# chiefchewie/thu-acg-f2024-path-tracer

Hardware: AMD Instinct MI355X
Metric: Msamples/s (WxHxspp/s), scene 6 FHD@4000spp (higher is better)
Workload: dtype f64; 1 GPU; scene 6 (reference main.rs scene script: bunny+spot+cow OBJ meshes, envmap) 1920x1080 @ 4000 spp, max_depth 50, seed 1; parallelism=single GPU (1-rank communicator, no collective), slots_per_pixel=0, device= (gfx950:sramecc+:xnack-)

## Files before the change

include/pt_amd.h:

```cpp
#ifndef PT_AMD_H
#define PT_AMD_H
#include <stdint.h>
#ifdef __cplusplus
extern "C" {
#endif

typedef struct pt_ctx pt_ctx;
typedef struct pt_scene pt_scene;

typedef struct pt_camera {
    double aspect_ratio;
    uint32_t image_width, samples_per_pixel, max_depth, env_is_map;
    double vfov;
    double look_from[3], look_at[3], vup[3];
    double blur_strength, focal_length, defocus_angle;
    double env_color[3];
    int32_t env_tex;
    int32_t _pad;
} pt_camera;

typedef struct pt_render_opts {
    uint32_t slots_per_pixel;
    uint32_t accum_on_device;
    uint32_t profile;
    uint32_t overwrite;
    void* stream;
} pt_render_opts;

typedef struct pt_render_stats {
    uint64_t samples, segments, iterations;
    uint32_t n_slots, slots_per_pixel;
    double ms_total;
    double ms_extend, ms_shade, ms_other;
    uint64_t launches_extend, launches_shade;
    uint32_t extend_variant, shade_variant;
    uint32_t blocks_extend, blocks_shade;
    uint32_t compactions;
    uint32_t n_alloc_end;
    uint64_t short_direct_tiles, short_self_prims;
    uint64_t short_walks, short_walk_passes;
    uint64_t pilot_tiles, short_fallback, short_list_bytes, short_pixels;
    double ms_pilot;
    uint64_t short_tiles, short_samples, hard_samples;
    double ms_short;
    uint64_t sky_tiles, sky_samples;
    double ms_sky;
} pt_render_stats;

const char* pt_last_error(void);
int pt_set_error_message(const char* msg);
int pt_ctx_create(int device, pt_ctx** out);
void pt_ctx_destroy(pt_ctx*);
int pt_device_name(pt_ctx*, char* buf, uint32_t n);
// ... 236 lines not shown
```

thu-acg-f2024-path-tracer_amd/__init__.py:

```python
from __future__ import annotations

import ctypes as C
import math
import os
from typing import Optional, Sequence

import numpy as np

_HERE = os.path.dirname(os.path.abspath(__file__))
REPO_ROOT = os.path.dirname(_HERE)
LIB_PATH = os.environ.get("PT_AMD_LIB") or os.path.join(_HERE, "libpt_amd.so")
ASSET_DIR = os.path.join(REPO_ROOT, "assets")


class PtError(RuntimeError):
    pass


class Camera(C.Structure):

    _fields_ = [
        ("aspect_ratio", C.c_double),
        ("image_width", C.c_uint32),
        ("samples_per_pixel", C.c_uint32),
# ... 29 lines not shown
        ("iterations", C.c_uint64),
        ("n_slots", C.c_uint32),
        ("slots_per_pixel", C.c_uint32),
        ("ms_total", C.c_double),
        ("ms_extend", C.c_double),
        ("ms_shade", C.c_double),
        ("ms_other", C.c_double),
        ("launches_extend", C.c_uint64),
        ("launches_shade", C.c_uint64),
        ("extend_variant", C.c_uint32),
        ("shade_variant", C.c_uint32),
        ("blocks_extend", C.c_uint32),
        ("blocks_shade", C.c_uint32),
        ("compactions", C.c_uint32),
        ("n_alloc_end", C.c_uint32),
        ("short_direct_tiles", C.c_uint64),
        ("short_self_prims", C.c_uint64),
        ("short_walks", C.c_uint64),
        ("short_walk_passes", C.c_uint64),
        ("pilot_tiles", C.c_uint64),
        ("short_fallback", C.c_uint64),
        ("short_list_bytes", C.c_uint64),
        ("short_pixels", C.c_uint64),
        ("ms_pilot", C.c_double),
        ("short_tiles", C.c_uint64),
        ("short_samples", C.c_uint64),
        ("hard_samples", C.c_uint64),
        ("ms_short", C.c_double),
        ("sky_tiles", C.c_uint64),
        ("sky_samples", C.c_uint64),
# ... 1181 lines not shown
```

thu-acg-f2024-path-tracer_amd/csrc/pt_k2.hip:

```cpp
#include "pt_k2_extend.h"

namespace pt {

typedef void (*extend_fn)(SceneD, PoolD, CountersD*);
static extend_fn pick_extend2(int code) {
    switch (code) {
    case 163: return k_extend2<16, 3>;
    case 164: return k_extend2<16, 4>;
    case 204: return k_extend2<20, 4>;
    case 283: return k_extend2<28, 3>;
    case 323: return k_extend2<32, 3>;
    case 1164: return k_extend2<16, 4, 64>;
    case 2164: return k_extend2<16, 4, 128>;
    case 8164: return k_extend2<16, 4, 512>;
    default: return k_extend2<24, 3>;
    }
}
static extend_fn pick_extend2_mot(int code) {
    const int stack = (code % 1000) / 10;
    if (stack <= 16) return k_extend2<16, 4, 128, true>;
    if (stack <= 20) return k_extend2<20, 4, BLOCK, true>;
    if (stack <= 24) return k_extend2<24, 3, BLOCK, true>;
    if (stack <= 28) return k_extend2<28, 3, BLOCK, true>;
    return k_extend2<32, 3, BLOCK, true>;
}
static int extend2_threads(int code) { return code >= 1000 ? (code / 1000) * 64 : BLOCK; }
static int extend2_threads_mot(int code) { return (code % 1000) / 10 <= 16 ? 128 : BLOCK; }
static extend_fn pick_extend_batch(uint32_t flat, uint32_t pairs, bool motion = false) {
    if (motion) return !flat ? k_extend<false, false, true> : pairs ? k_extend<true, true, true> : k_extend<true, false, true>;
    return !flat ? k_extend<false, false> : pairs ? k_extend<true, true> : k_extend<true, false>;
}
void launch_extend(const SceneD& sc, const PoolD& pool, CountersD* cnt, int max_blocks, int code, hipStream_t st, bool motion) {
    if (code <= -100) {
        const int kb = motion ? extend2_threads_mot(-code) : extend2_threads(-code);
        const uint32_t blocks = clamp_blocks(pool.n_alloc / (uint32_t)(EXT_WINDOW / BLOCK * kb), max_blocks);
        hipLaunchKernelGGL(motion ? pick_extend2_mot(-code) : pick_extend2(-code), dim3(blocks), dim3((uint32_t)kb), 0, st, sc, pool, cnt);
    }
    else hipLaunchKernelGGL(pick_extend_batch(sc.tlas_flat, sc.flat_pairs, motion), grid_for(pool.n_alloc, max_blocks), dim3(BLOCK), 0, st, sc, pool, cnt);
}
int extend_occupancy_blocks(int code, bool motion) {
    if (code <= -100) return motion ? occupancy_blocks((const void*)pick_extend2_mot(-code), extend2_threads_mot(-code))
                                    : occupancy_blocks((const void*)pick_extend2(-code), extend2_threads(-code));
    return occupancy_blocks((const void*)pick_extend_batch(code <= -2, code == -3, motion), BLOCK);
}

}
```

thu-acg-f2024-path-tracer_amd/csrc/pt_k2_extend.h:

```cpp
#pragma once
#include "pt_k_trace.h"

namespace pt {

#ifndef PT_EXTEND_BATCH_BLOCKS
#define PT_EXTEND_BATCH_BLOCKS 4
#endif

#ifndef PT_PAIR_DENSE_MIN
#define PT_PAIR_DENSE_MIN 16
#endif
#ifndef PT_PAIR_PASS_ATTR
#define PT_PAIR_PASS_ATTR PT_DEV
#endif
#ifndef PT_FLAT_DIRECT
#define PT_FLAT_DIRECT 1
#endif
#ifndef PT_CUBOID_CULL
#define PT_CUBOID_CULL 1
#endif
#ifndef PT_PAIR_SINGLE
#define PT_PAIR_SINGLE 1
#endif
constexpr int PAIR_CAP = 128;
// ... 203 lines not shown
constexpr int EXT_WINDOW = 2048;
#ifndef PT_REFILL_MIN
#define PT_REFILL_MIN 16
#endif
constexpr uint32_t REFILL_MIN = PT_REFILL_MIN;
#ifndef PT_EXT_CAND
#define PT_EXT_CAND 768
#endif
#ifndef PT_EXT_CAND_SMALL
#define PT_EXT_CAND_SMALL 1024
#endif
constexpr int EXT_CAND = PT_EXT_CAND, EXT_CAND_SMALL = PT_EXT_CAND_SMALL;
static_assert(EXT_WINDOW % BLOCK == 0 && EXT_WINDOW <= 65536, "k_extend2: s_cand_sl holds 16-bit slot offsets inside the window");
static_assert(EXT_WINDOW == SORT_WINDOW_SLOTS, "the pool is allocated in whole windows of this size (pt_render.cpp rounds n_alloc to 2048)");

template <int EXT_STACK, int MINB, int KB = BLOCK, bool MOT = false>
__global__ __launch_bounds__(KB, MINB) void k_extend2(SceneD sc, PoolD pool, CountersD* cnt) {
    constexpr int WIN = EXT_WINDOW / BLOCK * KB, CAND = (KB <= 128 ? EXT_CAND_SMALL : EXT_CAND) / BLOCK * KB;
    __shared__ uint32_t stack[EXT_STACK * KB];
    __shared__ uint32_t s_best_id[WIN];
    __shared__ double s_cand_t[CAND];
    __shared__ uint32_t s_cand_items[CAND];
    __shared__ uint16_t s_cand_sl[CAND];
    __shared__ uint32_t s_nrays, s_next, s_win;
    uint32_t* stk = &stack[threadIdx.x];
    const int lane = (int)(threadIdx.x & 63u);
    const double t_min = 1e-3;
    const float t_min_f = __double2float_rd(t_min);
    unsigned long long nseg = 0;
    const uint32_t n_windows = pool.n_alloc / WIN;
    constexpr uint32_t PARTS = PT_TAIL_SPLIT ? PT_TAIL_PARTS : 1, CH = (uint32_t)(WIN / KB) / PARTS;
    static_assert(PARTS * CH == (uint32_t)(WIN / KB), "");
    const uint32_t n_tail = PT_TAIL_SPLIT ? (n_windows < gridDim.x * PT_TAIL_SPAN ? n_windows : gridDim.x * PT_TAIL_SPAN) : 0u;
    const uint32_t n_full = n_windows - n_tail, n_queue = n_full + PARTS * n_tail;
    if (blockIdx.x == 0 && threadIdx.x == 0) cnt->win_shade = 0;
    if (ldu(&cnt->alive) == 0ull) return;
#ifdef PT_STAMPS
    if (threadIdx.x < 8) g_prof[CLASS_DEAD][threadIdx.x] = 0ull;
#endif
    if (threadIdx.x == 0) { s_win = (uint32_t)atomicAdd(&cnt->win_extend, 1ull); s_nrays = 0; s_next = 0; }
    __syncthreads();
    for (;;) {
        const uint32_t q = s_win;
        if (q >= n_queue) break;
        const uint32_t win = q < n_full ? q : n_full + (q - n_full) / PARTS;
        const int j_lo = q < n_full ? 0 : (int)(((q - n_full) % PARTS) * CH), j_hi = q < n_full ? WIN / KB : j_lo + (int)CH;
        const uint32_t wbase = (PT_K2_REVERSE ? n_windows - 1u - win : win) * WIN;
        PT_STAMP(e0);
#if PT_K2_PREFETCH
        uint32_t state_next = pool.bounce[wbase + (uint32_t)j_lo * KB + threadIdx.x];
        RayD r_next{};
        if (state_next < SLOT_IDLE) r_next = load_ray(pool, wbase + (uint32_t)j_lo * KB + threadIdx.x);
#endif
        for (int j = j_lo; j < j_hi; ++j) {
            const uint32_t sl = (uint32_t)j * KB + threadIdx.x;
#if PT_K2_PREFETCH
            const uint32_t state = state_next;
            const bool alive = state < SLOT_IDLE;
            const RayD r = r_next;
            if (j + 1 < j_hi) {
                state_next = pool.bounce[wbase + sl + KB];
                if (state_next < SLOT_IDLE) r_next = load_ray(pool, wbase + sl + KB);
            }
#else
            const uint32_t state = pool.bounce[wbase + sl];
            const bool alive = state < SLOT_IDLE;
            RayD r{};
            if (alive) r = load_ray(pool, wbase + sl);
#endif
            uint32_t n_my = 0, items = 0xFFFFFFFFu;
            RayF f{};
            Closest best{D_INF, HIT_NONE};
            float t_max_f = t_max_f32(best.t);
            if (alive) {
                ++nseg;
                f = make_rayf(r.o, r.d, sc.tlas_extent);
            }
            auto visit_entry = [&](auto uniform, uint32_t ei, const Entry& e, int sp) {
                constexpr bool U = decltype(uniform)::value;
                if (e.kind == ENTRY_MESH) {
                    if (n_my < 4u && ei < 0xFFu) {
                        items = (items & ~(0xFFu << (8u * n_my))) | (ei << (8u * n_my));
                        ++n_my;
                    } else {
                        blas_pass<KB, MOT>(sc, r, e, t_min, t_min_f, stk + (size_t)sp * KB, EXT_STACK - sp, best);
                        t_max_f = t_max_f32(best.t);
                    }
                } else {
                    const RayD lr = ray_to_local_chain<U, MOT>(sc, e.inst, r);
                    const uint32_t n = e.kind == ENTRY_CUBOID ? 6u : 1u;
                    for (uint32_t i = 0; i < n; ++i) test_world_prim<U>(sc, lr, t_min, e.first_prim + i, best);
                    t_max_f = t_max_f32(best.t);
                }
            };
            if (sc.tlas_flat) {
                best = flat_top_level<false, true, MOT>(sc, alive, r, f, t_min, t_min_f, lane, PairLds{}, [&](uint32_t ei, const Entry& e, Closest& b) {
                    best = b;
                    visit_entry(std::true_type{}, ei, e, 0);
                    b = best;
                });
            } else if (alive) {
                int sp = 0;
                uint32_t cur = sc.tlas_root;
                for (;;) {
                    if ((cur & REF_TYPE_MASK) == REF_NODE) {
                        uint32_t c0, c1;
                        const int n = visit_node(&sc.nodes[cur], f, t_min_f, t_max_f, c0, c1);
                        if (n == 2 && sp < EXT_STACK) stk[(sp++) * KB] = c1;
                        if (n > 0) {
                            cur = c0;
                            continue;
                        }
                    } else if ((cur & REF_TYPE_MASK) == REF_ENTRY) {
                        const uint32_t ei = cur & 0x3FFFFFFFu;
                        visit_entry(std::false_type{}, ei, sc.entries[ei], sp);
                    }
                    if (sp == 0) break;
                    cur = stk[(--sp) * KB];
                }
            }
            const unsigned long long m = __ballot(n_my > 0);
            if (m) {
                const int leader = __ffsll((long long)m) - 1;
                uint32_t base = 0;
                if (lane == leader) base = atomicAdd(&s_nrays, (uint32_t)__popcll(m));
                base = (uint32_t)__shfl((int)base, leader);
                if (n_my > 0) {
                    const uint32_t pos = base + (uint32_t)__popcll(m & ((1ull << lane) - 1ull));
                    if (pos < (uint32_t)CAND) {
                        s_cand_t[pos] = best.t;
                        s_cand_items[pos] = items;
                        s_cand_sl[pos] = (uint16_t)sl;
                    } else {
                        for (uint32_t k = 0; k < n_my; ++k) blas_pass<KB, MOT>(sc, r, sc.entries[(items >> (8u * k)) & 0xFFu], t_min, t_min_f, stk, EXT_STACK, best);
                    }
                }
            }
            s_best_id[sl] = alive ? best.id : dead_or_idle(state);
        }
        PT_STAMP(e1);
        __syncthreads();
        PT_STAMP(e2);
        const uint32_t n_rays = s_nrays < (uint32_t)CAND ? s_nrays : (uint32_t)CAND;
        {
            bool busy = false, exhausted = false;
            uint32_t sl = 0, items = 0, item_k = 0, cur = REF_EMPTY, first_prim = 0;
            int sp = 0;
            RayD wr{}, r{};
            RayF f{};
            Closest best{D_INF, HIT_NONE};
            float t_max_f = 0.0f;
            auto start_item = [&]() -> bool {
                const uint32_t ei = item_k < 4u ? (items >> (8u * item_k)) & 0xFFu : 0xFFu;
                if (ei == 0xFFu) return false;
                const Entry e = sc.entries[ei];
                r = ray_to_local_chain<false, MOT>(sc, e.inst, wr);
                first_prim = e.first_prim;
                f = make_rayf(r.o, r.d, e.extent);
                t_max_f = t_max_f32(best.t);
// ... 37 lines not shown
                    if ((cur & REF_TYPE_MASK) == REF_TRIS) {
                        const uint32_t first = cur & 0x07FFFFFFu, count = ((cur >> 27) & 7u) + 1u;
                        test_leaf(sc, first, count, r, t_min, first_prim, best);
                        t_max_f = t_max_f32(best.t);
                        cur = sp > 0 ? stk[(--sp) * KB] : REF_EMPTY;
                    }
                    if (cur == REF_EMPTY) {
                        ++item_k;
                        if (!start_item()) {
                            s_best_id[sl] = best.id;
                            busy = false;
                        }
                    }
                }
            }
        }
        PT_STAMP(e3);
        __syncthreads();
        PT_STAMP(e4);
#ifdef PT_STAMPS
        if (lane == 0) {
            atomicAdd(&g_prof[CLASS_DEAD][0], 1ull);
            atomicAdd(&g_prof[CLASS_DEAD][1], t_e1 - t_e0);
            atomicAdd(&g_prof[CLASS_DEAD][2], t_e2 - t_e1);
            atomicAdd(&g_prof[CLASS_DEAD][3], t_e3 - t_e2);
            atomicAdd(&g_prof[CLASS_DEAD][4], t_e4 - t_e3);
            atomicAdd(&g_prof[CLASS_DEAD][5], (unsigned long long)n_rays);
        }
#endif
        {
            uint32_t word[WIN / KB];
#pragma unroll
            for (int j = 0; j < WIN / KB; ++j) word[j] = (j >= j_lo && j < j_hi) ? hit_word(sc, s_best_id[(uint32_t)j * KB + threadIdx.x]) : 0u;
#pragma unroll
            for (int j = 0; j < WIN / KB; ++j) if (j >= j_lo && j < j_hi) stnt(&pool.hit_prim[wbase + (uint32_t)j * KB + threadIdx.x], word[j]);
        }
        if (threadIdx.x == 0) { s_win = (uint32_t)atomicAdd(&cnt->win_extend, 1ull); s_nrays = 0; s_next = 0; }
        __syncthreads();
    }
    nseg = wave_sum(nseg);
    if (nseg && (threadIdx.x & 63u) == 0u) atomicAdd(&cnt->segments, nseg);
#ifdef PT_STAMPS
    __syncthreads();
    if (threadIdx.x < 8 && g_prof[CLASS_DEAD][threadIdx.x]) atomicAdd(&cnt->prof[CLASS_DEAD][threadIdx.x], g_prof[CLASS_DEAD][threadIdx.x]);
#endif
}

}
```

thu-acg-f2024-path-tracer_amd/csrc/pt_kernels.h:

```cpp
#pragma once
#include <hip/hip_runtime_api.h>

#include "pt_types.h"

namespace pt {
struct ShadeForm { int variant = 0; bool lights = false, list = false, qmc = false; ShadeMode mode = MODE_PLAIN; bool motion = false, punctual = false; };
ShadeForm shade_form(ShadeForm asked);
bool shade_form_sorts(const ShadeForm& form);
bool shade_form_maps_tiles(const ShadeForm& form);
bool launch_init(const CamD& cam, const PoolD& pool, uint64_t seed, int max_blocks, hipStream_t st, const ShadeForm& form);
void launch_extend(const SceneD& sc, const PoolD& pool, CountersD* cnt, int max_blocks, int code, hipStream_t st, bool motion = false);
bool launch_shade(const SceneD& sc, const CamD& cam, const PoolD& pool, CountersD* cnt, uint64_t seed, int max_blocks, const ShadeForm& form, hipStream_t st,
                  uint32_t wide_window_min = 16, const EnvTabD* env = nullptr);
int extend_occupancy_blocks(int code, bool motion = false);
int shade_occupancy_blocks(const ShadeForm& form);
void launch_medium_probe(int which, double density, double g, const double* in, uint32_t n, double* out, hipStream_t st);
void launch_grid_probe(int which, const GridD* grid, const float* vals, const double* in, uint32_t n, double* out, hipStream_t st);
void launch_absorb_probe(const double absorption[3], const double* in, uint32_t n, double* out, hipStream_t st);
void launch_light_probe(const SceneD& sc, bool exact, int which, const double* in, uint32_t n, double* out, hipStream_t st);
void launch_dispersion_probe(int kind, int which, uint64_t seed, double n_d, double b, double inv2_d, const double* w, const double* in, uint32_t n, double* out, hipStream_t st);
void launch_sampler_probe(int kind, uint64_t seed, uint32_t pixel, uint32_t sample_begin, uint32_t n_samples, uint32_t draw_begin, uint32_t n_draws, uint64_t* out,
                          hipStream_t st);
void launch_env_tables(const SceneD& sc, const TexD& tex, double* col, double* row, hipStream_t st);
void launch_env_probe(const SceneD& sc, const TexD& tex, const EnvTabD& e, int which, const double* in, uint32_t n, double* out, hipStream_t st);
void launch_resolve(const PoolD& pool, double* accum, int max_blocks, hipStream_t st);
void launch_compact(const PoolD& pool, uint32_t new_end, uint32_t* holes, uint32_t* movers, uint32_t* counts, uint32_t cap, int max_blocks, hipStream_t st);
// ... 33 lines not shown
```

thu-acg-f2024-path-tracer_amd/csrc/pt_render.cpp:

```cpp
#include <hip/hip_runtime.h>

#include <algorithm>
#include <chrono>
#include <cmath>
#include <cstdio>
#include <cstdlib>
#include <cstring>
#include <vector>

#include "../../include/pt_amd.h"
#include "pt_kernels.h"
#include "pt_scene.h"
#include "pt_sky_tiles.h"

using namespace pt;
using namespace pt::host;

extern "C" const char* pt_last_error(void) { return pt::last_error(); }
extern "C" int pt_set_error_message(const char* msg) { return set_error(msg); }

extern "C" int pt_ctx_create(int device, pt_ctx** out) {
    *out = nullptr;
    int n = 0;
    if (hipGetDeviceCount(&n) != hipSuccess || n <= 0)
// ... 362 lines not shown
    bool pool_slots_set = false;
    uint64_t pool_slots = 0;
    int shade_variant = 42;
    bool pool_in_place = false, no_defer_regen = false, no_compact_records = false, init_shuffle = false, accum_linear = false, no_compact_pool = false,
         prof = false, no_sky_pass = false, no_short_pass = false;
    uint64_t short_cap_bytes = 0;
    bool no_pilot = false, pilot_any_range = false, pilot_margin_set = false, pilot_narrow = false;
    double pilot_theta = PILOT_THETA, pilot_margin = 1.5;
    uint32_t walk_cap = SHORT_WALK_STACK;
    bool no_short_defer = false;
    uint32_t short_chunk_mult = 4;
    bool no_short_reach = false, no_short_direct = false, no_short_self = false;
    int grid_mult = 1;
    uint32_t wide_window_min = 16;
    int ext2 = 0;
    enum { K2_AUTO, K2_BATCH, K2_TWOPHASE } k2 = K2_AUTO;
    uint64_t compact_num = 1, compact_den = 2;
    uint32_t poll_cap = 8;
};
Switches read_switches(const pt_render_opts& opts) {
    Switches sw;
    sw.slots_per_pixel = opts.slots_per_pixel;
    if (sw.slots_per_pixel == 0)
        if (const char* e = exp_env("PT_SLOTS_PER_PIXEL")) sw.slots_per_pixel = (uint32_t)atoi(e);
    if (const char* e = exp_env("PT_POOL_SLOTS")) {
        sw.pool_slots_set = true;
        sw.pool_slots = strtoull(e, nullptr, 10);
    }
    if (const char* e = exp_env("PT_SHADE_VARIANT")) sw.shade_variant = atoi(e);
    sw.pool_in_place = exp_env("PT_POOL_IN_PLACE") != nullptr;
    sw.no_defer_regen = exp_env("PT_NO_DEFER_REGEN") != nullptr;
    sw.no_compact_records = exp_env("PT_NO_COMPACT_RECORDS") != nullptr;
    sw.init_shuffle = exp_env("PT_INIT_SHUFFLE") != nullptr;
    if (const char* e = exp_env("PT_GRID_MULT")) sw.grid_mult = std::max(1, atoi(e));
    if (const char* e = exp_env("PT_WIDE_WINDOW_MIN")) sw.wide_window_min = (uint32_t)std::max(1, atoi(e));
    if (const char* e = exp_env("PT_EXT2")) sw.ext2 = atoi(e);
    if (const char* e = exp_env("PT_K2")) sw.k2 = !strcmp(e, "batch") ? Switches::K2_BATCH : !strcmp(e, "twophase") ? Switches::K2_TWOPHASE : Switches::K2_AUTO;
    sw.accum_linear = exp_env("PT_ACCUM_LINEAR") != nullptr;
    sw.no_compact_pool = exp_env("PT_NO_COMPACT_POOL") != nullptr;
    if (const char* e = exp_env("PT_COMPACT_AT")) { sw.compact_num = (uint64_t)std::max(1, atoi(e)); sw.compact_den = 100; }
    if (const char* e = exp_env("PT_POLL_CAP")) sw.poll_cap = (uint32_t)std::max(1, atoi(e));
    sw.prof = exp_env("PT_PROF") != nullptr;
    if (const char* e = exp_env("PT_SKY_PASS")) sw.no_sky_pass = atoi(e) == 0;
    if (const char* e = exp_env("PT_SHORT_PASS")) sw.no_short_pass = atoi(e) == 0;
    if (const char* e = exp_env("PT_SHORT_CAP_BYTES")) sw.short_cap_bytes = strtoull(e, nullptr, 10);
    if (const char* e = exp_env("PT_SHORT_PILOT")) sw.no_pilot = atoi(e) == 0;
    if (const char* e = exp_env("PT_PILOT_ANY_RANGE")) sw.pilot_any_range = atoi(e) != 0;
    if (const char* e = exp_env("PT_PILOT_THETA")) sw.pilot_theta = atof(e);
    if (const char* e = exp_env("PT_PILOT_MARGIN")) { sw.pilot_margin_set = true; sw.pilot_margin = std::max(0.0, atof(e)); }
    if (const char* e = exp_env("PT_PILOT_STACK")) sw.walk_cap = (uint32_t)std::min<int>(SHORT_WALK_STACK, std::max(0, atoi(e)));
    if (const char* e = exp_env("PT_PILOT_NARROW")) sw.pilot_narrow = atoi(e) != 0;
// ... 362 lines not shown
        if (c / 10 >= need && (c == 163 || c == 164 || c == 204 || c == 243 || c == 283 || c == 323)) code = c;
        if ((c == 1164 || c == 2164 || c == 8164) && need <= 16) code = c;
    }
    return code;
}
Kernels choose_kernels(const Switches& sw, const pt_scene* s, const Job& job, const PoolPlan& p) {
    Kernels kn;
    kn.form = job.form;
    kn.ordered = p.dynamic && !job.list && shade_form_sorts(kn.form) && !sw.pool_in_place;
    const int two_phase = extend2_code(s, sw);
    kn.extend_code = (s->n_mesh_entries > 0 && two_phase != 0) ? -two_phase : -1;
    if (sw.k2 == Switches::K2_BATCH) kn.extend_code = -1;
    else if (sw.k2 == Switches::K2_TWOPHASE && two_phase != 0) kn.extend_code = -two_phase;
    const int blocks_extend = extend_occupancy_blocks(kn.extend_code == -1 && s->dev.view.tlas_flat ? (s->dev.view.flat_pairs ? -3 : -2) : kn.extend_code, kn.form.motion);
    kn.blocks_shade = shade_occupancy_blocks(kn.form);
    kn.grid_extend = s->ctx->n_cus * blocks_extend * sw.grid_mult;
    kn.grid_shade = s->ctx->n_cus * kn.blocks_shade * sw.grid_mult;
    return kn;
}

int bind_pool(pt_scene* s, const Switches& sw, const Job& job, const PoolPlan& p, const Kernels& kn, PoolD& pool) {
    const size_t n_al = ((size_t)p.n_slots + 8191) & ~(size_t)8191;
    const size_t n_f64 = p.dynamic ? 0 : 6;
    const size_t bytes = n_al * (sizeof(RayRec) + sizeof(PathRec) + n_f64 * sizeof(double) + 2 * sizeof(uint32_t)) +
                         (kn.ordered ? n_al * (sizeof(RayRec) + sizeof(PathRec) + sizeof(uint32_t)) : 0);
    if (!s->pool_mem.reserve(bytes, "hipMalloc(path pool)")) return -1;
    if (!s->d_counters) {
        if (!hip_ok(hipMalloc((void**)&s->d_counters, sizeof(CountersD)), "hipMalloc(counters)")) return -1;
        if (!hip_ok(hipHostMalloc((void**)&s->h_counters, sizeof(CountersD), hipHostMallocDefault), "hipHostMalloc(counters)")) return -1;
    }
    memset(&pool, 0, sizeof pool);
// ... 101 lines not shown
    }
    const bool wavefront = !(job.sky && job.n_active_tiles == 0);
    if (wavefront) {
        timer.begin(2, st);
        if (!launch_init(dc, pool, job.seed, kn.grid_shade, st, kn.form)) return set_error("pt_render: no k_init form for this render");
        timer.end(st);
    }
    const uint64_t per_slot = p.dynamic ? (p.total_work + p.n_slots - 1) / std::max<uint64_t>(p.n_slots, 1) + 1 : (job.spp + p.k - 1) / p.k;
    const uint64_t max_iterations = per_slot * ((uint64_t)std::max(1u, dc.max_depth) + 1) + 4;
    uint32_t poll_every = 8;
    const bool compact_ok = p.dynamic && !sw.no_compact_pool;
    bool alive = job.spp != 0 && dc.max_depth != 0 && wavefront;
    while (alive) {
        for (uint32_t i = 0; i < poll_every; ++i) {
            timer.begin(0, st);
            launch_extend(s->dev.view, pool, s->d_counters, kn.grid_extend, kn.extend_code, st, kn.form.motion);
            timer.end(st);
            timer.begin(1, st);
            if (!launch_shade(s->dev.view, dc, pool, s->d_counters, job.seed, kn.grid_shade, kn.form, st, sw.wide_window_min, mode_has_table(job.mode) ? &job.env : nullptr))
                return set_error("pt_render: no k_shade form for this render");
            timer.end(st);
            if (kn.ordered) {
                std::swap(pool.ray, pool.ray_out);
                std::swap(pool.path, pool.path_out);
                std::swap(pool.bounce, pool.bounce_out);
            }
            ++r.iterations;
        }
        if (!hip_ok(hipMemcpyAsync(s->h_counters, s->d_counters, sizeof(CountersD), hipMemcpyDeviceToHost, st), "hipMemcpy(counters)")) return -1;
        if (!hip_ok(hipStreamSynchronize(st), "hipStreamSynchronize(render)")) return -1;
        timer.drain();
// ... 31 lines not shown
                const size_t j = 3 * (size_t)job.h_list[i] + c;
                accum[j] = job.opts.overwrite ? tmp[j] : accum[j] + tmp[j];
            }
    } else {
        for (size_t i = 0; i < n; ++i) accum[i] += tmp[i];
    }
    return 0;
}

void print_prof(const CountersD* cnt) {
    static const char* names[N_CLASSES + 1] = {"miss", "diffuse", "metal", "glass", "principled", "light", "sheen", "clearcoat", "mix", "idle", "dead", "WINDOW"};
    for (uint32_t c = 0; c <= N_CLASSES; ++c) {
        const unsigned long long* p = cnt->prof[c];
        if (p[0] && c == CLASS_DEAD)
            fprintf(stderr, "[pt prof] K2 window  n %10llu  phase A %8.0f  barrier %8.0f  phase B %8.0f  barrier %8.0f  candidates %6.1f (cycles per window and wave)\n", p[0],
                    (double)p[1] / p[0], (double)p[2] / p[0], (double)p[3] / p[0], (double)p[4] / p[0], (double)p[5] / p[0]);
        else if (p[0] && c < N_CLASSES)
            fprintf(stderr, "[pt prof] %-10s n %10llu  body %8.0f = hit %7.0f + env/tex %7.0f + direction %7.0f + pdf/eval/ray %7.0f  dequeue %8.0f  regen+store %8.0f  whole %8.0f (cycles per wave-group)\n",
                    names[c], p[0], (double)p[2] / p[0], (double)p[1] / p[0], (double)p[6] / p[0], (double)p[7] / p[0], (double)(p[2] - p[1] - p[6] - p[7]) / p[0],
                    (double)p[3] / p[0], (double)p[4] / p[0], (double)p[5] / p[0]),
            fprintf(stderr, "[pt prof] %-10s   lanes per group: live %5.1f  on a surface %5.1f  with a next direction %5.1f  regenerated %5.1f\n", names[c], (double)p[8] / p[0],
                    (double)p[9] / p[0], (double)p[10] / p[0], (double)p[11] / p[0])
#ifdef PT_STAMPS
            , fprintf(stderr, "[pt prof] %-10s   groups of one primitive %10llu (%5.1f %%), of one sphere / quad %10llu (%5.1f %%)\n", names[c], p[12], 100.0 * (double)p[12] / p[0],
                      p[13], 100.0 * (double)p[13] / p[0])
#endif
            ;
        else if (p[0])
            fprintf(stderr, "[pt prof] WINDOW     n %10llu  sort %8.0f  shade %8.0f  barrier wait %8.0f  groups %8.0f  record wait %8.0f (cycles per window and wave)\n", p[0],
                    (double)p[1] / p[0], (double)p[2] / p[0], (double)p[3] / p[0], (double)p[4] / p[0], (double)p[5] / p[0]);
    }
// ... 6 lines not shown
    stats->iterations = r.iterations;
    stats->n_slots = p.n_slots;
    stats->slots_per_pixel = p.dynamic ? 0u : p.k;
    stats->ms_total = r.ms_total;
    stats->ms_extend = timer.ms[0];
    stats->ms_shade = timer.ms[1];
    stats->ms_other = timer.ms[2];
    stats->launches_extend = timer.launches[0];
    stats->launches_shade = timer.launches[1];
    stats->extend_variant = kn.extend_code <= -100 ? 0u : 1u;
    stats->shade_variant = (uint32_t)kn.form.variant;
    stats->blocks_extend = (uint32_t)kn.grid_extend;
    stats->blocks_shade = (uint32_t)kn.grid_shade;
    stats->compactions = r.compactions;
    stats->n_alloc_end = pool.n_alloc;
    stats->pilot_tiles = job.n_pilot_tiles;
    stats->short_fallback = job.short_fallback ? 1u : 0u;
    stats->short_list_bytes = job.n_short_tiles ? job.short_cap_entries * (job.short_wide ? 8 : 4) : 0u;
    stats->short_pixels = job.n_short_pixels;
    stats->short_direct_tiles = job.short_direct_tiles;
    stats->short_self_prims = job.n_short_tiles ? job.short_self_prims : 0u;
    stats->short_walks = job.short_walks;
    stats->short_walk_passes = job.short_walk_passes;
    stats->ms_pilot = timer.ms[5];
    stats->short_tiles = job.n_short_tiles;
    stats->short_samples = job.short_samples;
    stats->hard_samples = job.n_hard;
    stats->ms_short = timer.ms[4];
    stats->sky_tiles = job.sky ? job.n_sky_tiles : 0u;
    stats->sky_samples = job.sky ? (uint64_t)job.n_sky_pixels * job.spp : 0u;
// ... 4 lines not shown
    sum.segments += ps.segments;
    sum.iterations += ps.iterations;
    sum.n_slots = std::max(sum.n_slots, ps.n_slots);
    sum.slots_per_pixel = ps.slots_per_pixel;
    sum.ms_extend += ps.ms_extend;
    sum.ms_shade += ps.ms_shade;
    sum.ms_other += ps.ms_other;
    sum.launches_extend += ps.launches_extend;
    sum.launches_shade += ps.launches_shade;
    sum.extend_variant = ps.extend_variant;
    sum.shade_variant = ps.shade_variant;
    sum.blocks_extend = ps.blocks_extend;
    sum.blocks_shade = ps.blocks_shade;
    sum.compactions += ps.compactions;
    sum.n_alloc_end = ps.n_alloc_end;
    sum.pilot_tiles = std::max(sum.pilot_tiles, ps.pilot_tiles);
    sum.short_fallback += ps.short_fallback;
    sum.short_list_bytes = std::max(sum.short_list_bytes, ps.short_list_bytes);
    sum.short_pixels = std::max(sum.short_pixels, ps.short_pixels);
    sum.short_direct_tiles = std::max(sum.short_direct_tiles, ps.short_direct_tiles);
    sum.short_self_prims = std::max(sum.short_self_prims, ps.short_self_prims);
    sum.short_walks += ps.short_walks;
    sum.short_walk_passes += ps.short_walk_passes;
    sum.ms_pilot += ps.ms_pilot;
    sum.short_tiles = std::max(sum.short_tiles, ps.short_tiles);
    sum.short_samples += ps.short_samples;
    sum.hard_samples += ps.hard_samples;
    sum.ms_short += ps.ms_short;
    sum.sky_tiles = std::max(sum.sky_tiles, ps.sky_tiles);
    sum.sky_samples += ps.sky_samples;
// ... 231 lines not shown
```

thu-acg-f2024-path-tracer_amd/csrc/pt_types.h:

```cpp
#pragma once
#include <stddef.h>
#include <stdint.h>

namespace pt {

struct alignas(16) BvhNode {
    float lo0[3], hi0[3];
    float lo1[3], hi1[3];
    uint32_t child0, child1;
    uint32_t pad0, pad1;
};
constexpr uint32_t REF_TYPE_MASK = 0xC0000000u;
constexpr uint32_t REF_NODE = 0x00000000u;
constexpr uint32_t REF_TRIS = 0x40000000u;
constexpr uint32_t REF_ENTRY = 0x80000000u;
constexpr uint32_t REF_EMPTY = 0xFFFFFFFFu;
constexpr uint32_t REF_LEAVE_INSTANCE = 0xC0000000u;
constexpr int TRAVERSAL_STACK = 32;
constexpr int MAX_BLAS_DEPTH = 20;
constexpr int MAX_TLAS_DEPTH = 10;

enum PrimKind : uint32_t { PRIM_SPHERE = 0, PRIM_QUAD = 1, PRIM_TRI = 2 };
enum EntryKind : uint32_t { ENTRY_SPHERE = 0, ENTRY_QUAD = 1, ENTRY_CUBOID = 2, ENTRY_MESH = 3 };
constexpr uint32_t PRIM_HAS_NORMALS = 1u << 8, PRIM_HAS_UVS = 1u << 9;
// ... 239 lines not shown
constexpr uint32_t SHORT_WORDS = 40, SHORT_PROF_AT = 8;
constexpr uint32_t SHORT_WALK_STACK = 16;
constexpr uint32_t SHORT_YIELD_BINS = 17;

constexpr uint32_t WORK_SHARDS = 64;
#ifdef PT_STAMPS
constexpr int PROF_COLS = 14;
#else
constexpr int PROF_COLS = 12;
#endif
struct CountersD {
    unsigned long long alive;
    unsigned long long segments;
    unsigned long long samples;
    unsigned long long win_extend, win_shade;
    unsigned long long pad[11];
    unsigned long long prof[N_CLASSES + 1][PROF_COLS];
    struct alignas(128) Shard { unsigned long long next; unsigned long long pad[15]; } work[WORK_SHARDS];
};

}
```

Baseline: 4297 Msamples/s.

## Split k_extend2 windows into segments to flush mesh candidates before overflow

New measurement: 4416 Msamples/s (median of 6 runs). 2.7% higher.

```diff
diff --git a/include/pt_amd.h b/include/pt_amd.h
--- a/include/pt_amd.h
+++ b/include/pt_amd.h
@@ -37,6 +37,7 @@
     uint32_t blocks_extend, blocks_shade;
     uint32_t compactions;
     uint32_t n_alloc_end;
+    uint64_t k2_split_windows, k2_overflow_rays;
     uint64_t short_direct_tiles, short_self_prims;
     uint64_t short_walks, short_walk_passes;
     uint64_t pilot_tiles, short_fallback, short_list_bytes, short_pixels;
diff --git a/thu-acg-f2024-path-tracer_amd/__init__.py b/thu-acg-f2024-path-tracer_amd/__init__.py
--- a/thu-acg-f2024-path-tracer_amd/__init__.py
+++ b/thu-acg-f2024-path-tracer_amd/__init__.py
@@ -67,6 +67,8 @@
         ("blocks_shade", C.c_uint32),
         ("compactions", C.c_uint32),
         ("n_alloc_end", C.c_uint32),
+        ("k2_split_windows", C.c_uint64),
+        ("k2_overflow_rays", C.c_uint64),
         ("short_direct_tiles", C.c_uint64),
         ("short_self_prims", C.c_uint64),
         ("short_walks", C.c_uint64),
diff --git a/thu-acg-f2024-path-tracer_amd/csrc/pt_k2.hip b/thu-acg-f2024-path-tracer_amd/csrc/pt_k2.hip
--- a/thu-acg-f2024-path-tracer_amd/csrc/pt_k2.hip
+++ b/thu-acg-f2024-path-tracer_amd/csrc/pt_k2.hip
@@ -3,7 +3,8 @@
 namespace pt {
 
 typedef void (*extend_fn)(SceneD, PoolD, CountersD*);
-static extend_fn pick_extend2(int code) {
+typedef void (*extend2_fn)(SceneD, PoolD, CountersD*, uint32_t);
+static extend2_fn pick_extend2(int code) {
     switch (code) {
     case 163: return k_extend2<16, 3>;
     case 164: return k_extend2<16, 4>;
@@ -16,7 +17,7 @@
     default: return k_extend2<24, 3>;
     }
 }
-static extend_fn pick_extend2_mot(int code) {
+static extend2_fn pick_extend2_mot(int code) {
     const int stack = (code % 1000) / 10;
     if (stack <= 16) return k_extend2<16, 4, 128, true>;
     if (stack <= 20) return k_extend2<20, 4, BLOCK, true>;
@@ -30,11 +31,11 @@
     if (motion) return !flat ? k_extend<false, false, true> : pairs ? k_extend<true, true, true> : k_extend<true, false, true>;
     return !flat ? k_extend<false, false> : pairs ? k_extend<true, true> : k_extend<true, false>;
 }
-void launch_extend(const SceneD& sc, const PoolD& pool, CountersD* cnt, int max_blocks, int code, hipStream_t st, bool motion) {
+void launch_extend(const SceneD& sc, const PoolD& pool, CountersD* cnt, int max_blocks, int code, hipStream_t st, bool motion, uint32_t split) {
     if (code <= -100) {
         const int kb = motion ? extend2_threads_mot(-code) : extend2_threads(-code);
         const uint32_t blocks = clamp_blocks(pool.n_alloc / (uint32_t)(EXT_WINDOW / BLOCK * kb), max_blocks);
-        hipLaunchKernelGGL(motion ? pick_extend2_mot(-code) : pick_extend2(-code), dim3(blocks), dim3((uint32_t)kb), 0, st, sc, pool, cnt);
+        hipLaunchKernelGGL(motion ? pick_extend2_mot(-code) : pick_extend2(-code), dim3(blocks), dim3((uint32_t)kb), 0, st, sc, pool, cnt, split);
     }
     else hipLaunchKernelGGL(pick_extend_batch(sc.tlas_flat, sc.flat_pairs, motion), grid_for(pool.n_alloc, max_blocks), dim3(BLOCK), 0, st, sc, pool, cnt);
 }
diff --git a/thu-acg-f2024-path-tracer_amd/csrc/pt_k2_extend.h b/thu-acg-f2024-path-tracer_amd/csrc/pt_k2_extend.h
--- a/thu-acg-f2024-path-tracer_amd/csrc/pt_k2_extend.h
+++ b/thu-acg-f2024-path-tracer_amd/csrc/pt_k2_extend.h
@@ -241,15 +241,22 @@
 static_assert(EXT_WINDOW % BLOCK == 0 && EXT_WINDOW <= 65536, "k_extend2: s_cand_sl holds 16-bit slot offsets inside the window");
 static_assert(EXT_WINDOW == SORT_WINDOW_SLOTS, "the pool is allocated in whole windows of this size (pt_render.cpp rounds n_alloc to 2048)");
 
+#ifdef PT_STAMPS
+#define K2_LAP(acc) do { const unsigned long long t_now = stamp(); acc += t_now - t_lap; t_lap = t_now; } while (0)
+#else
+#define K2_LAP(acc)
+#endif
+constexpr uint32_t K2_SPLIT_OFF = 0, K2_SPLIT_HALF = 1, K2_SPLIT_DRAIN = 2;
 template <int EXT_STACK, int MINB, int KB = BLOCK, bool MOT = false>
-__global__ __launch_bounds__(KB, MINB) void k_extend2(SceneD sc, PoolD pool, CountersD* cnt) {
+__global__ __launch_bounds__(KB, MINB) void k_extend2(SceneD sc, PoolD pool, CountersD* cnt, uint32_t split) {
     constexpr int WIN = EXT_WINDOW / BLOCK * KB, CAND = (KB <= 128 ? EXT_CAND_SMALL : EXT_CAND) / BLOCK * KB;
+    constexpr int NSEG = WIN / KB + 1;
     __shared__ uint32_t stack[EXT_STACK * KB];
     __shared__ uint32_t s_best_id[WIN];
     __shared__ double s_cand_t[CAND];
     __shared__ uint32_t s_cand_items[CAND];
     __shared__ uint16_t s_cand_sl[CAND];
-    __shared__ uint32_t s_nrays, s_next, s_win;
+    __shared__ uint32_t s_seg[NSEG], s_next, s_win, s_stat[2];
     uint32_t* stk = &stack[threadIdx.x];
     const int lane = (int)(threadIdx.x & 63u);
     const double t_min = 1e-3;
@@ -263,9 +270,10 @@
     if (blockIdx.x == 0 && threadIdx.x == 0) cnt->win_shade = 0;
     if (ldu(&cnt->alive) == 0ull) return;
 #ifdef PT_STAMPS
-    if (threadIdx.x < 8) g_prof[CLASS_DEAD][threadIdx.x] = 0ull;
-#endif
-    if (threadIdx.x == 0) { s_win = (uint32_t)atomicAdd(&cnt->win_extend, 1ull); s_nrays = 0; s_next = 0; }
+    if (threadIdx.x < PROF_COLS) g_prof[CLASS_DEAD][threadIdx.x] = 0ull;
+#endif
+    if (threadIdx.x == 0) { s_win = (uint32_t)atomicAdd(&cnt->win_extend, 1ull); s_next = 0; s_stat[0] = 0; s_stat[1] = 0; }
+    if (threadIdx.x < (uint32_t)NSEG) s_seg[threadIdx.x] = 0;
     __syncthreads();
     for (;;) {
         const uint32_t q = s_win;
@@ -273,103 +281,14 @@
         const uint32_t win = q < n_full ? q : n_full + (q - n_full) / PARTS;
         const int j_lo = q < n_full ? 0 : (int)(((q - n_full) % PARTS) * CH), j_hi = q < n_full ? WIN / KB : j_lo + (int)CH;
         const uint32_t wbase = (PT_K2_REVERSE ? n_windows - 1u - win : win) * WIN;
-        PT_STAMP(e0);
-#if PT_K2_PREFETCH
-        uint32_t state_next = pool.bounce[wbase + (uint32_t)j_lo * KB + threadIdx.x];
-        RayD r_next{};
-        if (state_next < SLOT_IDLE) r_next = load_ray(pool, wbase + (uint32_t)j_lo * KB + threadIdx.x);
-#endif
-        for (int j = j_lo; j < j_hi; ++j) {
-            const uint32_t sl = (uint32_t)j * KB + threadIdx.x;
-#if PT_K2_PREFETCH
-            const uint32_t state = state_next;
-            const bool alive = state < SLOT_IDLE;
-            const RayD r = r_next;
-            if (j + 1 < j_hi) {
-                state_next = pool.bounce[wbase + sl + KB];
-                if (state_next < SLOT_IDLE) r_next = load_ray(pool, wbase + sl + KB);
-            }
-#else
-            const uint32_t state = pool.bounce[wbase + sl];
-            const bool alive = state < SLOT_IDLE;
-            RayD r{};
-            if (alive) r = load_ray(pool, wbase + sl);
-#endif
-            uint32_t n_my = 0, items = 0xFFFFFFFFu;
-            RayF f{};
-            Closest best{D_INF, HIT_NONE};
-            float t_max_f = t_max_f32(best.t);
-            if (alive) {
-                ++nseg;
-                f = make_rayf(r.o, r.d, sc.tlas_extent);
-            }
-            auto visit_entry = [&](auto uniform, uint32_t ei, const Entry& e, int sp) {
-                constexpr bool U = decltype(uniform)::value;
-                if (e.kind == ENTRY_MESH) {
-                    if (n_my < 4u && ei < 0xFFu) {
-                        items = (items & ~(0xFFu << (8u * n_my))) | (ei << (8u * n_my));
-                        ++n_my;
-                    } else {
-                        blas_pass<KB, MOT>(sc, r, e, t_min, t_min_f, stk + (size_t)sp * KB, EXT_STACK - sp, best);
-                        t_max_f = t_max_f32(best.t);
-                    }
-                } else {
-                    const RayD lr = ray_to_local_chain<U, MOT>(sc, e.inst, r);
-                    const uint32_t n = e.kind == ENTRY_CUBOID ? 6u : 1u;
-                    for (uint32_t i = 0; i < n; ++i) test_world_prim<U>(sc, lr, t_min, e.first_prim + i, best);
-                    t_max_f = t_max_f32(best.t);
-                }
-            };
-            if (sc.tlas_flat) {
-                best = flat_top_level<false, true, MOT>(sc, alive, r, f, t_min, t_min_f, lane, PairLds{}, [&](uint32_t ei, const Entry& e, Closest& b) {
-                    best = b;
-                    visit_entry(std::true_type{}, ei, e, 0);
-                    b = best;
-                });
-            } else if (alive) {
-                int sp = 0;
-                uint32_t cur = sc.tlas_root;
-                for (;;) {
-                    if ((cur & REF_TYPE_MASK) == REF_NODE) {
-                        uint32_t c0, c1;
-                        const int n = visit_node(&sc.nodes[cur], f, t_min_f, t_max_f, c0, c1);
-                        if (n == 2 && sp < EXT_STACK) stk[(sp++) * KB] = c1;
-                        if (n > 0) {
-                            cur = c0;
-                            continue;
-                        }
-                    } else if ((cur & REF_TYPE_MASK) == REF_ENTRY) {
-                        const uint32_t ei = cur & 0x3FFFFFFFu;
-                        visit_entry(std::false_type{}, ei, sc.entries[ei], sp);
-                    }
-                    if (sp == 0) break;
-                    cur = stk[(--sp) * KB];
-                }
-            }
-            const unsigned long long m = __ballot(n_my > 0);
-            if (m) {
-                const int leader = __ffsll((long long)m) - 1;
-                uint32_t base = 0;
-                if (lane == leader) base = atomicAdd(&s_nrays, (uint32_t)__popcll(m));
-                base = (uint32_t)__shfl((int)base, leader);
-                if (n_my > 0) {
-                    const uint32_t pos = base + (uint32_t)__popcll(m & ((1ull << lane) - 1ull));
-                    if (pos < (uint32_t)CAND) {
-                        s_cand_t[pos] = best.t;
-                        s_cand_items[pos] = items;
-                        s_cand_sl[pos] = (uint16_t)sl;
-                    } else {
-                        for (uint32_t k = 0; k < n_my; ++k) blas_pass<KB, MOT>(sc, r, sc.entries[(items >> (8u * k)) & 0xFFu], t_min, t_min_f, stk, EXT_STACK, best);
-                    }
-                }
-            }
-            s_best_id[sl] = alive ? best.id : dead_or_idle(state);
-        }
-        PT_STAMP(e1);
-        __syncthreads();
-        PT_STAMP(e2);
-        const uint32_t n_rays = s_nrays < (uint32_t)CAND ? s_nrays : (uint32_t)CAND;
-        {
+        const int j_rule = q >= n_full || split == K2_SPLIT_OFF ? j_hi : split == K2_SPLIT_HALF ? j_lo + (j_hi - j_lo) / 2 : CAND / KB;
+        const uint32_t n_rule = split == K2_SPLIT_HALF ? (uint32_t)CAND / 2u : (uint32_t)(CAND - KB);
+        uint32_t n_list = 0, seg = 0;
+#ifdef PT_STAMPS
+        unsigned long long t_lap = stamp(), p_a = 0, p_wa = 0, p_b = 0, p_wb = 0, p_over = 0;
+        uint32_t n_walked = 0, n_window = 0;
+#endif
+        auto phase_b = [&](const uint32_t n_rays) {
             bool busy = false, exhausted = false;
             uint32_t sl = 0, items = 0, item_k = 0, cur = REF_EMPTY, first_prim = 0;
             int sp = 0;
@@ -437,18 +356,143 @@
                     }
                 }
             }
-        }
-        PT_STAMP(e3);
+        };
+#if PT_K2_PREFETCH
+        uint32_t state_next = pool.bounce[wbase + (uint32_t)j_lo * KB + threadIdx.x];
+        RayD r_next{};
+        if (state_next < SLOT_IDLE) r_next = load_ray(pool, wbase + (uint32_t)j_lo * KB + threadIdx.x);
+#endif
+        for (int j = j_lo; j < j_hi; ++j) {
+            const uint32_t sl = (uint32_t)j * KB + threadIdx.x;
+#if PT_K2_PREFETCH
+            const uint32_t state = state_next;
+            const bool alive = state < SLOT_IDLE;
+            const RayD r = r_next;
+            if (j + 1 < j_hi) {
+                state_next = pool.bounce[wbase + sl + KB];
+                if (state_next < SLOT_IDLE) r_next = load_ray(pool, wbase + sl + KB);
+            }
+#else
+            const uint32_t state = pool.bounce[wbase + sl];
+            const bool alive = state < SLOT_IDLE;
+            RayD r{};
+            if (alive) r = load_ray(pool, wbase + sl);
+#endif
+            uint32_t n_my = 0, items = 0xFFFFFFFFu;
+            RayF f{};
+            Closest best{D_INF, HIT_NONE};
+            float t_max_f = t_max_f32(best.t);
+            if (alive) {
+                ++nseg;
+                f = make_rayf(r.o, r.d, sc.tlas_extent);
+            }
+            auto visit_entry = [&](auto uniform, uint32_t ei, const Entry& e, int sp) {
+                constexpr bool U = decltype(uniform)::value;
+                if (e.kind == ENTRY_MESH) {
+                    if (n_my < 4u && ei < 0xFFu) {
+                        items = (items & ~(0xFFu << (8u * n_my))) | (ei << (8u * n_my));
+                        ++n_my;
+                    } else {
+                        blas_pass<KB, MOT>(sc, r, e, t_min, t_min_f, stk + (size_t)sp * KB, EXT_STACK - sp, best);
+                        t_max_f = t_max_f32(best.t);
+                    }
+                } else {
+                    const RayD lr = ray_to_local_chain<U, MOT>(sc, e.inst, r);
+                    const uint32_t n = e.kind == ENTRY_CUBOID ? 6u : 1u;
+                    for (uint32_t i = 0; i < n; ++i) test_world_prim<U>(sc, lr, t_min, e.first_prim + i, best);
+                    t_max_f = t_max_f32(best.t);
+                }
+            };
+            if (sc.tlas_flat) {
+                best = flat_top_level<false, true, MOT>(sc, alive, r, f, t_min, t_min_f, lane, PairLds{}, [&](uint32_t ei, const Entry& e, Closest& b) {
+                    best = b;
+                    visit_entry(std::true_type{}, ei, e, 0);
+                    b = best;
+                });
+            } else if (alive) {
+                int sp = 0;
+                uint32_t cur = sc.tlas_root;
+                for (;;) {
+                    if ((cur & REF_TYPE_MASK) == REF_NODE) {
+                        uint32_t c0, c1;
+                        const int n = visit_node(&sc.nodes[cur], f, t_min_f, t_max_f, c0, c1);
+                        if (n == 2 && sp < EXT_STACK) stk[(sp++) * KB] = c1;
+                        if (n > 0) {
+                            cur = c0;
+                            continue;
+                        }
+                    } else if ((cur & REF_TYPE_MASK) == REF_ENTRY) {
+                        const uint32_t ei = cur & 0x3FFFFFFFu;
+                        visit_entry(std::false_type{}, ei, sc.entries[ei], sp);
+                    }
+                    if (sp == 0) break;
+                    cur = stk[(--sp) * KB];
+                }
+            }
+            const unsigned long long m = __ballot(n_my > 0);
+            if (m) {
+                const int leader = __ffsll((long long)m) - 1;
+                uint32_t base = 0;
+                if (lane == leader) base = atomicAdd(&s_seg[seg], (uint32_t)__popcll(m));
+                base = n_list + (uint32_t)__shfl((int)base, leader);
+#ifdef PT_STAMPS
+                const bool walks = __ballot(n_my > 0 && base + (uint32_t)__popcll(m & ((1ull << lane) - 1ull)) >= (uint32_t)CAND) != 0ull;
+                const unsigned long long t_walk = walks ? stamp() : 0ull;
+#endif
+                if (n_my > 0) {
+                    const uint32_t pos = base + (uint32_t)__popcll(m & ((1ull << lane) - 1ull));
+                    if (pos < (uint32_t)CAND) {
+                        s_cand_t[pos] = best.t;
+                        s_cand_items[pos] = items;
+                        s_cand_sl[pos] = (uint16_t)sl;
+                    } else {
+                        for (uint32_t k = 0; k < n_my; ++k) blas_pass<KB, MOT>(sc, r, sc.entries[(items >> (8u * k)) & 0xFFu], t_min, t_min_f, stk, EXT_STACK, best);
+                    }
+                }
+#ifdef PT_STAMPS
+                if (walks) p_over += stamp() - t_walk;
+#endif
+            }
+            s_best_id[sl] = alive ? best.id : dead_or_idle(state);
+            const int jn = j + 1;
+            const bool last = jn == j_hi;
+            if (!last && !(split == K2_SPLIT_DRAIN ? jn >= j_rule : jn == j_rule)) continue;
+            K2_LAP(p_a);
+            __syncthreads();
+            K2_LAP(p_wa);
+            n_list += (uint32_t)__builtin_amdgcn_readfirstlane((int)s_seg[seg]);
+            ++seg;
+            if (!last && n_list <= n_rule) continue;
+            const uint32_t n_over = n_list > (uint32_t)CAND ? n_list - (uint32_t)CAND : 0u;
+            if (threadIdx.x == 0) { s_stat[0] += last ? 0u : 1u; s_stat[1] += n_over; }
+#ifdef PT_STAMPS
+            n_walked += n_over;
+            n_window += n_list;
+#endif
+            phase_b(n_list - n_over);
+            K2_LAP(p_b);
+            if (last) break;
+            __syncthreads();
+            K2_LAP(p_wb);
+            if (threadIdx.x == 0) s_next = 0;
+            n_list = 0;
+        }
         __syncthreads();
-        PT_STAMP(e4);
+        K2_LAP(p_wb);
 #ifdef PT_STAMPS
         if (lane == 0) {
             atomicAdd(&g_prof[CLASS_DEAD][0], 1ull);
-            atomicAdd(&g_prof[CLASS_DEAD][1], t_e1 - t_e0);
-            atomicAdd(&g_prof[CLASS_DEAD][2], t_e2 - t_e1);
-            atomicAdd(&g_prof[CLASS_DEAD][3], t_e3 - t_e2);
-            atomicAdd(&g_prof[CLASS_DEAD][4], t_e4 - t_e3);
-            atomicAdd(&g_prof[CLASS_DEAD][5], (unsigned long long)n_rays);
+            atomicAdd(&g_prof[CLASS_DEAD][1], p_a);
+            atomicAdd(&g_prof[CLASS_DEAD][2], p_wa);
+            atomicAdd(&g_prof[CLASS_DEAD][3], p_b);
+            atomicAdd(&g_prof[CLASS_DEAD][4], p_wb);
+            atomicAdd(&g_prof[CLASS_DEAD][5], (unsigned long long)(n_window - n_walked));
+            atomicAdd(&g_prof[CLASS_DEAD][7], p_over);
+        }
+        if (threadIdx.x == 0) {
+            atomicAdd(&g_prof[CLASS_DEAD][6], (unsigned long long)n_walked);
+            const uint32_t bin = n_window * 8u / (uint32_t)WIN;
+            if (q < n_full) atomicAdd(&g_prof[CLASS_DEAD][8 + bin / 2u], 1ull << (32u * (bin & 1u)));
         }
 #endif
         {
@@ -458,15 +502,20 @@
 #pragma unroll
             for (int j = 0; j < WIN / KB; ++j) if (j >= j_lo && j < j_hi) stnt(&pool.hit_prim[wbase + (uint32_t)j * KB + threadIdx.x], word[j]);
         }
-        if (threadIdx.x == 0) { s_win = (uint32_t)atomicAdd(&cnt->win_extend, 1ull); s_nrays = 0; s_next = 0; }
+        if (threadIdx.x == 0) { s_win = (uint32_t)atomicAdd(&cnt->win_extend, 1ull); s_next = 0; }
+        if (threadIdx.x < (uint32_t)NSEG) s_seg[threadIdx.x] = 0;
         __syncthreads();
     }
     nseg = wave_sum(nseg);
     if (nseg && (threadIdx.x & 63u) == 0u) atomicAdd(&cnt->segments, nseg);
+    if (threadIdx.x == 0) {
+        if (s_stat[0]) atomicAdd(&cnt->k2_split_windows, (unsigned long long)s_stat[0]);
+        if (s_stat[1]) atomicAdd(&cnt->k2_overflow_rays, (unsigned long long)s_stat[1]);
+    }
 #ifdef PT_STAMPS
     __syncthreads();
-    if (threadIdx.x < 8 && g_prof[CLASS_DEAD][threadIdx.x]) atomicAdd(&cnt->prof[CLASS_DEAD][threadIdx.x], g_prof[CLASS_DEAD][threadIdx.x]);
-#endif
-}
-
-}
+    if (threadIdx.x < PROF_COLS && g_prof[CLASS_DEAD][threadIdx.x]) atomicAdd(&cnt->prof[CLASS_DEAD][threadIdx.x], g_prof[CLASS_DEAD][threadIdx.x]);
+#endif
+}
+
+}
diff --git a/thu-acg-f2024-path-tracer_amd/csrc/pt_kernels.h b/thu-acg-f2024-path-tracer_amd/csrc/pt_kernels.h
--- a/thu-acg-f2024-path-tracer_amd/csrc/pt_kernels.h
+++ b/thu-acg-f2024-path-tracer_amd/csrc/pt_kernels.h
@@ -9,7 +9,7 @@
 bool shade_form_sorts(const ShadeForm& form);
 bool shade_form_maps_tiles(const ShadeForm& form);
 bool launch_init(const CamD& cam, const PoolD& pool, uint64_t seed, int max_blocks, hipStream_t st, const ShadeForm& form);
-void launch_extend(const SceneD& sc, const PoolD& pool, CountersD* cnt, int max_blocks, int code, hipStream_t st, bool motion = false);
+void launch_extend(const SceneD& sc, const PoolD& pool, CountersD* cnt, int max_blocks, int code, hipStream_t st, bool motion = false, uint32_t split = 1);
 bool launch_shade(const SceneD& sc, const CamD& cam, const PoolD& pool, CountersD* cnt, uint64_t seed, int max_blocks, const ShadeForm& form, hipStream_t st,
                   uint32_t wide_window_min = 16, const EnvTabD* env = nullptr);
 int extend_occupancy_blocks(int code, bool motion = false);
diff --git a/thu-acg-f2024-path-tracer_amd/csrc/pt_render.cpp b/thu-acg-f2024-path-tracer_amd/csrc/pt_render.cpp
--- a/thu-acg-f2024-path-tracer_amd/csrc/pt_render.cpp
+++ b/thu-acg-f2024-path-tracer_amd/csrc/pt_render.cpp
@@ -400,6 +400,8 @@
     int grid_mult = 1;
     uint32_t wide_window_min = 16;
     int ext2 = 0;
+    uint32_t k2_split = 1;
+    int k2_blocks = 0;
     enum { K2_AUTO, K2_BATCH, K2_TWOPHASE } k2 = K2_AUTO;
     uint64_t compact_num = 1, compact_den = 2;
     uint32_t poll_cap = 8;
@@ -421,6 +423,8 @@
     if (const char* e = exp_env("PT_GRID_MULT")) sw.grid_mult = std::max(1, atoi(e));
     if (const char* e = exp_env("PT_WIDE_WINDOW_MIN")) sw.wide_window_min = (uint32_t)std::max(1, atoi(e));
     if (const char* e = exp_env("PT_EXT2")) sw.ext2 = atoi(e);
+    if (const char* e = exp_env("PT_K2_SPLIT")) sw.k2_split = (uint32_t)std::min(2, std::max(0, atoi(e)));
+    if (const char* e = exp_env("PT_K2_BLOCKS")) sw.k2_blocks = std::max(0, atoi(e));
     if (const char* e = exp_env("PT_K2")) sw.k2 = !strcmp(e, "batch") ? Switches::K2_BATCH : !strcmp(e, "twophase") ? Switches::K2_TWOPHASE : Switches::K2_AUTO;
     sw.accum_linear = exp_env("PT_ACCUM_LINEAR") != nullptr;
     sw.no_compact_pool = exp_env("PT_NO_COMPACT_POOL") != nullptr;
@@ -813,7 +817,7 @@
     else if (sw.k2 == Switches::K2_TWOPHASE && two_phase != 0) kn.extend_code = -two_phase;
     const int blocks_extend = extend_occupancy_blocks(kn.extend_code == -1 && s->dev.view.tlas_flat ? (s->dev.view.flat_pairs ? -3 : -2) : kn.extend_code, kn.form.motion);
     kn.blocks_shade = shade_occupancy_blocks(kn.form);
-    kn.grid_extend = s->ctx->n_cus * blocks_extend * sw.grid_mult;
+    kn.grid_extend = sw.k2_blocks ? sw.k2_blocks : s->ctx->n_cus * blocks_extend * sw.grid_mult;
     kn.grid_shade = s->ctx->n_cus * kn.blocks_shade * sw.grid_mult;
     return kn;
 }
@@ -945,7 +949,7 @@
     while (alive) {
         for (uint32_t i = 0; i < poll_every; ++i) {
             timer.begin(0, st);
-            launch_extend(s->dev.view, pool, s->d_counters, kn.grid_extend, kn.extend_code, st, kn.form.motion);
+            launch_extend(s->dev.view, pool, s->d_counters, kn.grid_extend, kn.extend_code, st, kn.form.motion, sw.k2_split);
             timer.end(st);
             timer.begin(1, st);
             if (!launch_shade(s->dev.view, dc, pool, s->d_counters, job.seed, kn.grid_shade, kn.form, st, sw.wide_window_min, mode_has_table(job.mode) ? &job.env : nullptr))
@@ -1007,7 +1011,14 @@
         const unsigned long long* p = cnt->prof[c];
         if (p[0] && c == CLASS_DEAD)
             fprintf(stderr, "[pt prof] K2 window  n %10llu  phase A %8.0f  barrier %8.0f  phase B %8.0f  barrier %8.0f  candidates %6.1f (cycles per window and wave)\n", p[0],
-                    (double)p[1] / p[0], (double)p[2] / p[0], (double)p[3] / p[0], (double)p[4] / p[0], (double)p[5] / p[0]);
+                    (double)p[1] / p[0], (double)p[2] / p[0], (double)p[3] / p[0], (double)p[4] / p[0], (double)p[5] / p[0])
+#ifdef PT_STAMPS
+            , fprintf(stderr, "[pt prof] K2 overflow  wave cycles: phase A %llu (of it chunk ends with a walk %llu)  barriers %llu  phase B %llu  barriers %llu; rays: phase B %llu (per wave-window sums: x waves per block)  walked in phase A %llu\n",
+                      p[1], p[7], p[2], p[3], p[4], p[5], p[6]),
+              fprintf(stderr, "[pt prof] K2 full windows by candidates in eighths of the window, 0 .. 8: %llu %llu %llu %llu %llu %llu %llu %llu %llu\n", p[8] & 0xFFFFFFFFull,
+                      p[8] >> 32, p[9] & 0xFFFFFFFFull, p[9] >> 32, p[10] & 0xFFFFFFFFull, p[10] >> 32, p[11] & 0xFFFFFFFFull, p[11] >> 32, p[12] & 0xFFFFFFFFull)
+#endif
+            ;
         else if (p[0] && c < N_CLASSES)
             fprintf(stderr, "[pt prof] %-10s n %10llu  body %8.0f = hit %7.0f + env/tex %7.0f + direction %7.0f + pdf/eval/ray %7.0f  dequeue %8.0f  regen+store %8.0f  whole %8.0f (cycles per wave-group)\n",
                     names[c], p[0], (double)p[2] / p[0], (double)p[1] / p[0], (double)p[6] / p[0], (double)p[7] / p[0], (double)(p[2] - p[1] - p[6] - p[7]) / p[0],
@@ -1044,6 +1055,8 @@
     stats->blocks_shade = (uint32_t)kn.grid_shade;
     stats->compactions = r.compactions;
     stats->n_alloc_end = pool.n_alloc;
+    stats->k2_split_windows = s->h_counters->k2_split_windows;
+    stats->k2_overflow_rays = s->h_counters->k2_overflow_rays;
     stats->pilot_tiles = job.n_pilot_tiles;
     stats->short_fallback = job.short_fallback ? 1u : 0u;
     stats->short_list_bytes = job.n_short_tiles ? job.short_cap_entries * (job.short_wide ? 8 : 4) : 0u;
@@ -1078,6 +1091,8 @@
     sum.blocks_shade = ps.blocks_shade;
     sum.compactions += ps.compactions;
     sum.n_alloc_end = ps.n_alloc_end;
+    sum.k2_split_windows += ps.k2_split_windows;
+    sum.k2_overflow_rays += ps.k2_overflow_rays;
     sum.pilot_tiles = std::max(sum.pilot_tiles, ps.pilot_tiles);
     sum.short_fallback += ps.short_fallback;
     sum.short_list_bytes = std::max(sum.short_list_bytes, ps.short_list_bytes);
diff --git a/thu-acg-f2024-path-tracer_amd/csrc/pt_types.h b/thu-acg-f2024-path-tracer_amd/csrc/pt_types.h
--- a/thu-acg-f2024-path-tracer_amd/csrc/pt_types.h
+++ b/thu-acg-f2024-path-tracer_amd/csrc/pt_types.h
@@ -277,7 +277,8 @@
     unsigned long long segments;
     unsigned long long samples;
     unsigned long long win_extend, win_shade;
-    unsigned long long pad[11];
+    unsigned long long k2_split_windows, k2_overflow_rays;
+    unsigned long long pad[9];
     unsigned long long prof[N_CLASSES + 1][PROF_COLS];
     struct alignas(128) Shard { unsigned long long next; unsigned long long pad[15]; } work[WORK_SHARDS];
 };
```
